# QZ1-boy/FCVSR

Hardware: AMD Instinct MI355X
Metric: SR frames/sec (7-frame window, 4x 180x320->720x1280) + PSNR vs ref (higher is better)
Workload: dtype bf16

## Files before the change

fcvsr_amd/csrc/iac.hip:

```cpp
#include "common.h"
#include "mfma_util.h"

namespace fcvsr {

typedef __attribute__((ext_vector_type(4))) float f32x4v_t;

constexpr int kIY = 4, kIX = 16, kIC = 32;
constexpr int kIHX = kIX + 2, kIHY = kIY + 2;

template <int KDT>
__device__ __forceinline__ void load_k12(const void* base, long long elem_off, float k[4][3]) {
  if (KDT == FCVSR_F32) {
    const float4* p = reinterpret_cast<const float4*>(reinterpret_cast<const float*>(base) + elem_off);
    const float4 a = p[0], b = p[1], c = p[2];
    k[0][0] = a.x; k[0][1] = a.y; k[0][2] = a.z; k[1][0] = a.w; k[1][1] = b.x; k[1][2] = b.y;
    k[2][0] = b.z; k[2][1] = b.w; k[2][2] = c.x; k[3][0] = c.y; k[3][1] = c.z; k[3][2] = c.w;
  } else {
    const uint2* p = reinterpret_cast<const uint2*>(reinterpret_cast<const uint16_t*>(base) + elem_off);
    const uint2 a = p[0], b = p[1], c = p[2];
    const unsigned w[6] = {a.x, a.y, b.x, b.y, c.x, c.y};
    float f[12];
#pragma unroll
    for (int i = 0; i < 6; ++i) {
      if (KDT == FCVSR_BF16) {
// ... 493 lines not shown
          for (int c = 0; c < 8; ++c) acc[c] = fmaf(v[c], k[c * 3 + tt], acc[c]);
        }
#pragma unroll
        for (int c = 0; c < 8; ++c) {
          acc[c] += f[c];
          acc[c] = acc[c] >= 0.f ? acc[c] : acc[c] * slope;
        }
        st_p8<ADT>(dst.p, (long long)b * dst.sb + (long long)gy * dst.sy + (long long)gx * dst.sx + c0, acc);
      }
    }
  };

  issue_taps(0);
  if (FK) {
    predictor_gemm();
    __syncthreads();
#pragma unroll
    for (int j = 0; j < 2; ++j) {
      const int p = j * 32 + ps;
      const uint4* kq = reinterpret_cast<const uint4*>(kt_s + ((p >> 4) * kIHX + (p & 15) + 1) * kKtRow + oct * 24);
      kin[j].q[0] = kq[0]; kin[j].q[1] = kq[1]; kin[j].q[2] = kq[2];
    }
    if (ps < 8) {
      const uint4* kq = reinterpret_cast<const uint4*>(kt_s + ((ps >> 1) * kIHX + ((ps & 1) ? kIHX - 1 : 0)) * kKtRow + oct * 24);
      khal.q[0] = kq[0]; khal.q[1] = kq[1]; khal.q[2] = kq[2];
    }
    __syncthreads();
  }
  warp_store(0);
  if (ND > 1) { issue_taps(1); issue_fin(1); }
  if (t + 1 < t_end) off_next = load_off(t + 1, tid);
  __syncthreads();
  sac_phases(0);
  if (ND > 1) {
    warp_store(1);
    __syncthreads();
    sac_phases(1);
  }
  }
}


constexpr int kQX = 14, kQVX = 16, kQY = 4, kQSY = kQY + 2;
constexpr int kQNS = kQSY * kQVX, kQNV = kQY * kQVX;

template <bool BF16>
__device__ __forceinline__ f32x4v_t mfma16x(uint4 a, uint4 b, f32x4v_t c) {
  if (BF16)
    return __builtin_amdgcn_mfma_f32_16x16x32_bf16(__builtin_bit_cast(bf16x8_t, a), __builtin_bit_cast(bf16x8_t, b), c, 0, 0, 0);
  else
    return __builtin_amdgcn_mfma_f32_16x16x32_f16(__builtin_bit_cast(f16x8_t, a), __builtin_bit_cast(f16x8_t, b), c, 0, 0, 0);
}

struct Iac2Args {
  const uint16_t* prev[2];
  const float* off[2];
  const uint16_t* fin[2];
  uint16_t* dst[2];
  const uint16_t* k0;
  const uint16_t* wk;
  const float* kbias;
  long long prev_sb, off_sb, fin_sb, dst_sb, k0_sb;
  int prev_sy, prev_sx, off_sy, off_sx, off_sc, fin_sy, fin_sx, dst_sy, dst_sx, k0_sy, k0_sx;
  float slope;
  int H, W, tiles_x, tiles_y, ntiles;
};

#ifndef FCVSR_IAC2_WGS
#define FCVSR_IAC2_WGS 3
#endif
template <int KDT, int ADT>
__global__ __launch_bounds__(256, FCVSR_IAC2_WGS) void iac_fused2_kernel(Iac2Args a) {
  constexpr int NG = 1;
  static_assert(ADT != FCVSR_F32 && KDT != FCVSR_F32, "16-bit form");
  constexpr bool BF = KDT == FCVSR_BF16;
  constexpr int SPP = 32 * NG;
  constexpr int ND = 2, NP = (kQNS + SPP - 1) / SPP;
  constexpr int EARLY = 2;
  __shared__ __align__(16) float s_all[kQNS * kJC];
  __shared__ __align__(16) uint16_t w_s[3 * kJC * kJC];
  __shared__ __align__(16) float kb_s[3 * kJC];
  const float slope = a.slope;
  const int H = a.H, W = a.W, tiles_x = a.tiles_x, tiles_y = a.tiles_y;
  int t_begin, t_end;
  {
    const int g = blockIdx.x, nwg = gridDim.x, qq = nwg >> 3, rr = nwg & 7, xcd = g & 7, loc = g >> 3;
    const int ci = (xcd < rr ? xcd * (qq + 1) : rr * (qq + 1) + (xcd - rr) * qq) + loc;
    t_begin = (int)((long long)ci * a.ntiles / nwg);
    t_end = (int)((long long)(ci + 1) * a.ntiles / nwg);
  }
  {
    const int tid = threadIdx.x;
#pragma unroll
    for (int i = 0; i < 3 * kJC * kJC / 8 / (256 * NG); ++i) {
      const int idx = tid + 256 * NG * i, R = idx >> 3, seg = idx & 7;
      const int mt = R >> 4, r = R & 15, tp = mt >> 2, cb = mt & 3;
      const int orig = ((r >> 2) * 16 + cb * 4 + (r & 3)) * 3 + tp;
      *reinterpret_cast<uint4*>(w_s + R * kJC + ((seg ^ (R & 7)) << 3)) = *reinterpret_cast<const uint4*>(a.wk + orig * kJC + seg * 8);
    }
    if (tid < 3 * kJC) {
      const int mt = tid >> 4, r = tid & 15, tp = mt >> 2, cb = mt & 3;
      kb_s[tid] = a.kbias[((r >> 2) * 16 + cb * 4 + (r & 3)) * 3 + tp];
    }
    __syncthreads();
  }
  auto load_off = [&](const int tt, const int tidv) {
    const int lanev = tidv & 63, wavev = tidv >> 6;
    const int bb = tt / (tiles_x * tiles_y), tt2 = tt - bb * tiles_x * tiles_y;
    const int oy0 = (tt2 / tiles_x) * kQY, ox0 = (tt2 % tiles_x) * kQX;
    const int sdir = lanev >> 5, sit = (lanev >> 3) & 3, spl = lanev & 7;
    int hp = sit * SPP + wavev * 8 + spl;
    hp = hp < kQNS ? hp : kQNS - 1;
    const int hy = hp >> 4, hx = hp & 15;
    int gy = oy0 + hy - 1, gx = ox0 + hx - 1;
    gy = gy < 0 ? 0 : (gy > H - 1 ? H - 1 : gy);
    gx = gx < 0 ? 0 : (gx > W - 1 ? W - 1 : gx);
    const float* op = (sdir ? a.off[1] : a.off[0]) + (long long)bb * a.off_sb + (gy * a.off_sy + gx * a.off_sx);
    return make_float2(op[0], op[a.off_sc]);
  };
  const int wave_s = __builtin_amdgcn_readfirstlane((int)threadIdx.x >> 6);
  float* const s_s = s_all;
  float* const v_s = s_s;
  float2 off_next = make_float2(0.f, 0.f);
  if (t_begin < t_end) off_next = load_off(t_begin, (int)threadIdx.x);
  for (int t = t_begin; t < t_end; ++t) {
    int tid;
    asm volatile("v_mbcnt_lo_u32_b32 %0, -1, 0\n\tv_mbcnt_hi_u32_b32 %0, -1, %0\n\tv_lshl_add_u32 %0, %1, 6, %0" : "=&v"(tid) : "s"(wave_s));
    auto fresh = [&]() { int x = tid; asm volatile("" : "+v"(x)); return x; };
    const int wave = wave_s;
    const int b = t / (tiles_x * tiles_y);
    const int t2 = t - b * tiles_x * tiles_y;
    const int ty0 = (t2 / tiles_x) * kQY, tx0 = (t2 % tiles_x) * kQX;
    const int row = ty0 + wave;
    const int rowc = row > H - 1 ? H - 1 : row;
    auto col_of = [&](const int n_) { const int x = tx0 + n_ - 1; return x < 0 ? 0 : (x > W - 1 ? W - 1 : x); };
    auto ld16 = [](const void* base, const unsigned byte_off) {
      Pack8<ADT> r;
      r.a = *reinterpret_cast<const uint4*>(reinterpret_cast<const char*>(base) + byte_off);
      r.b = make_uint4(0, 0, 0, 0);
      return r;
    };
    uint4 kfr[2];
    {
      const int x = fresh(), n = x & 15, q = (x & 63) >> 4;
      const uint16_t* kb = a.k0 + (long long)b * a.k0_sb + (long long)rowc * a.k0_sy;
      const unsigned e = (unsigned)(col_of(n) * a.k0_sx + q * 8) * 2u;
      kfr[0] = ld16(kb, e).a;
      kfr[1] = ld16(kb, e + 64u).a;
    }
    int my_eo[4];
    float my_w[4];
    {
      const int x = fresh(), lane = x & 63;
      const int sit = (lane >> 3) & 3, spl = lane & 7;
      int hp = sit * SPP + wave * 8 + spl;
      hp = hp < kQNS ? hp : kQNS - 1;
      const int hy = hp >> 4, hx = hp & 15;
      int gy = ty0 + hy - 1, gx = tx0 + hx - 1;
      gy = gy < 0 ? 0 : (gy > H - 1 ? H - 1 : gy);
      gx = gx < 0 ? 0 : (gx > W - 1 ? W - 1 : gx);
      const int psy = a.prev_sy, psx = a.prev_sx;
      const float fx = (float)gx + off_next.x;
      const float fy = (float)gy + off_next.y;
      const float x0f = floorf(fx), y0f = floorf(fy);
      const float wx1 = fx - x0f, wy1 = fy - y0f;
      const float wx0 = 1.f - wx1, wy0 = 1.f - wy1;
      int wb, hb;
      asm volatile("v_mov_b32 %0, %2\n\tv_mov_b32 %1, %3" : "=&v"(wb), "=&v"(hb) : "s"(W + 1), "s"(H + 1));
      const bool sane = (fx > -2.f) && (fx < (float)wb) && (fy > -2.f) && (fy < (float)hb);
      const int x0 = sane ? (int)x0f : -4, y0 = sane ? (int)y0f : -4;
#pragma unroll
      for (int dy = 0; dy < 2; ++dy) {
#pragma unroll
        for (int dx = 0; dx < 2; ++dx) {
          const int xi = x0 + dx, yi = y0 + dy;
          const bool in = xi >= 0 && xi < W && yi >= 0 && yi < H;
          const int xc = xi < 0 ? 0 : (xi > W - 1 ? W - 1 : xi), yc = yi < 0 ? 0 : (yi > H - 1 ? H - 1 : yi);
          my_w[dy * 2 + dx] = in ? (dy ? wy1 : wy0) * (dx ? wx1 : wx0) : 0.f;
          my_eo[dy * 2 + dx] = yc * psy + xc * psx;
        }
      }
    }
    __builtin_amdgcn_sched_barrier(0);
    Pack8<ADT> fpk[2];
    auto issue_fin = [&](const int dir) {
      const int x = fresh(), n = x & 15, q = (x & 63) >> 4;
      const uint16_t* fb = a.fin[dir] + (long long)b * a.fin_sb + (long long)rowc * a.fin_sy;
      const unsigned e = (unsigned)(col_of(n) * a.fin_sx + q * 16) * 2u;
      fpk[0] = ld16(fb, e);
      fpk[1] = ld16(fb, e + 16u);
    };
    Pack8<ADT> tap[ND][NP][4];
    auto issue_taps = [&](const int dir, const int it0, const int it1) {
      const int x = fresh(), oct = x & 7, pull = ((x & 63) >> 3) << 2;
      const uint16_t* pb = a.prev[dir] + (long long)b * a.prev_sb;
#pragma unroll
      for (int it = it0; it < it1; ++it) {
        const int src = pull + dir * 128 + it * 32;
#pragma unroll
        for (int k = 0; k < 4; ++k)
          tap[dir][it][k] = ld16(pb, (unsigned)(__builtin_amdgcn_ds_bpermute(src, my_eo[k]) + oct * 8) * 2u);
      }
    };
    auto warp_store = [&](const int dir) {
      const int x = fresh(), oct = x & 7, ps = x >> 3, pull = ((x & 63) >> 3) << 2;
#pragma unroll
      for (int it = 0; it < NP; ++it) {
        const int hp = it * SPP + ps;
        const int src = pull + dir * 128 + it * 32;
        float acc[8] = {0.f, 0.f, 0.f, 0.f, 0.f, 0.f, 0.f, 0.f};
        float tw[4];
#pragma unroll
        for (int k = 0; k < 4; ++k) tw[k] = __int_as_float(__builtin_amdgcn_ds_bpermute(src, __float_as_int(my_w[k])));
#pragma unroll
        for (int k = 0; k < 4; ++k) {
          float v[8];
          unpack8<ADT>(tap[dir][it][k], v);
          const float w = tw[k];
#pragma unroll
          for (int c = 0; c < 8; ++c) acc[c] = fmaf(v[c], w, acc[c]);
        }
        float* rec = s_s + hp * kJC;
        if (kQNS % SPP == 0 || hp < kQNS) {
          *reinterpret_cast<float4*>(rec + (((2 * oct) ^ (hp & 15)) << 2)) = make_float4(acc[0], acc[1], acc[2], acc[3]);
          *reinterpret_cast<float4*>(rec + (((2 * oct + 1) ^ (hp & 15)) << 2)) = make_float4(acc[4], acc[5], acc[6], acc[7]);
        }
        __builtin_amdgcn_sched_barrier(0);
      }
    };
    issue_taps(0, 0, NP);
    __builtin_amdgcn_sched_barrier(0);
    constexpr bool KF = NG == 1 && BF;
    uint2 K1p[KF ? 1 : 12];
    float K1f[KF ? 12 : 1][4];
    {
      const int x = fresh(), n = x & 15, q = (x & 63) >> 4;
#pragma unroll
      for (int mt = 0; mt < 12; ++mt) {
        const int R = mt * 16 + n;
        const uint4 w0 = *reinterpret_cast<const uint4*>(w_s + R * kJC + ((q ^ (R & 7)) << 3));
        const uint4 w1 = *reinterpret_cast<const uint4*>(w_s + R * kJC + (((q + 4) ^ (R & 7)) << 3));
        f32x4v_t acc = {0.f, 0.f, 0.f, 0.f};
        acc = mfma16x<BF>(w0, kfr[0], acc);
        acc = mfma16x<BF>(w1, kfr[1], acc);
        const float4 b4 = *reinterpret_cast<const float4*>(kb_s + mt * 16 + q * 4);
        const uint2 pk = cvt4<BF>(make_float4(acc[0] + b4.x, acc[1] + b4.y, acc[2] + b4.z, acc[3] + b4.w));
        if (KF) cvt16x4_to_f32<BF>(pk, K1f[mt]);
        else K1p[mt] = pk;
        if (mt & 1) __builtin_amdgcn_sched_barrier(0);
      }
    }
    int ov[4], oh[3][4];
    {
      const int x = fresh(), n = x & 15, q = (x & 63) >> 4;
#pragma unroll
      for (int cb = 0; cb < 4; ++cb) {
        ov[cb] = n * kJC + (((q * 4 + cb) ^ n) << 2);
#pragma unroll
        for (int tt = 0; tt < 3; ++tt) {
          const int m = n + tt - 1;
          oh[tt][cb] = m * kJC + (((q * 4 + cb) ^ (m & 15)) << 2);
        }
      }
    }
    auto sac = [&](const int dir) {
      float4 vr[4];
      {
#pragma unroll
        for (int cb = 0; cb < 4; ++cb) {
          float acc[4] = {0.f, 0.f, 0.f, 0.f};
#pragma unroll
          for (int tt = 0; tt < 3; ++tt) {
            const float4 sv = *reinterpret_cast<const float4*>(s_s + (wave + tt) * (kQVX * kJC) + ov[cb]);
            float k[4];
            if (KF) { k[0] = K1f[tt * 4 + cb][0]; k[1] = K1f[tt * 4 + cb][1]; k[2] = K1f[tt * 4 + cb][2]; k[3] = K1f[tt * 4 + cb][3]; }
            else cvt16x4_to_f32<BF>(K1p[tt * 4 + cb], k);
            acc[0] = fmaf(sv.x, k[0], acc[0]); acc[1] = fmaf(sv.y, k[1], acc[1]);
            acc[2] = fmaf(sv.z, k[2], acc[2]); acc[3] = fmaf(sv.w, k[3], acc[3]);
          }
          vr[cb] = make_float4(acc[0], acc[1], acc[2], acc[3]);
          __builtin_amdgcn_sched_barrier(0);
        }
      }
      issue_fin(dir);
      __syncthreads();
#pragma unroll
      for (int cb = 0; cb < 4; ++cb) *reinterpret_cast<float4*>(v_s + wave * (kQVX * kJC) + ov[cb]) = vr[cb];
      __syncthreads();
      const int x = fresh(), n = x & 15, q = (x & 63) >> 4;
      const int gx = tx0 + n - 1;
      if (n >= 1 && n <= kQX && row < H && gx < W) {
        uint16_t* const db = a.dst[dir] + (long long)b * a.dst_sb + (long long)row * a.dst_sy;
        const int e = gx * a.dst_sx + q * 16;
#pragma unroll
        for (int hf = 0; hf < 2; ++hf) {
          float f[8], o[8];
          unpack8<ADT>(fpk[hf], f);
#pragma unroll
          for (int c2 = 0; c2 < 2; ++c2) {
            const int cb = hf * 2 + c2;
            float acc[4] = {0.f, 0.f, 0.f, 0.f};
#pragma unroll
            for (int tt = 0; tt < 3; ++tt) {
              const float4 vv = *reinterpret_cast<const float4*>(v_s + wave * (kQVX * kJC) + oh[tt][cb]);
              float k[4];
              if (KF) { k[0] = K1f[tt * 4 + cb][0]; k[1] = K1f[tt * 4 + cb][1]; k[2] = K1f[tt * 4 + cb][2]; k[3] = K1f[tt * 4 + cb][3]; }
              else cvt16x4_to_f32<BF>(K1p[tt * 4 + cb], k);
              acc[0] = fmaf(vv.x, k[0], acc[0]); acc[1] = fmaf(vv.y, k[1], acc[1]);
              acc[2] = fmaf(vv.z, k[2], acc[2]); acc[3] = fmaf(vv.w, k[3], acc[3]);
            }
#pragma unroll
            for (int i = 0; i < 4; ++i) {
              const float r = acc[i] + f[c2 * 4 + i];
              o[c2 * 4 + i] = fmaxf(r, r * slope);
            }
          }
          st_p8<ADT>(reinterpret_cast<float*>(db), e + hf * 8, o);
          __builtin_amdgcn_sched_barrier(0);
        }
      }
    };
    __builtin_amdgcn_sched_barrier(0);
    warp_store(0);
    __builtin_amdgcn_sched_barrier(0);
    issue_taps(1, 0, EARLY);
    __builtin_amdgcn_sched_barrier(0);
    __syncthreads();
    sac(0);
    issue_taps(1, EARLY, NP);
    if (t + 1 < t_end) off_next = load_off(t + 1, fresh());
    __builtin_amdgcn_sched_barrier(0);
    __syncthreads();
    warp_store(1);
    __syncthreads();
    sac(1);
    __syncthreads();
  }
}

}

using namespace fcvsr;

static bool quad_ok(const fcvsr_view* v, int dt) {
  if (!v || !v->ptr || v->dtype != dt || v->sc != 1 || v->c % 4) return false;
  const int g = dt == FCVSR_F32 ? 4 : 4;
  const int al = dt == FCVSR_F32 ? 16 : 8;
  return v->sx % g == 0 && v->sy % g == 0 && v->sb % g == 0 && ((uintptr_t)v->ptr % al) == 0;
}

static int iac_persistent_wgs() {
  static int n[64] = {0};
  int dev = 0;
  if (hipGetDevice(&dev) != hipSuccess || dev < 0 || dev >= 64) return 512;
  if (!n[dev]) {
    hipDeviceProp_t prop;
    n[dev] = hipGetDeviceProperties(&prop, dev) == hipSuccess && prop.multiProcessorCount > 0 ? 2 * prop.multiProcessorCount : 512;
  }
  return n[dev];
}

template <int KDT, int ND, bool FK = false>
static void launch_iac64(int adt, dim3 grid, hipStream_t st, IacArgs a) {
  a.ntiles = (int)grid.x;
  if (FK) {
    int nwg = iac_persistent_wgs() / (int)grid.y;
    nwg = nwg < 8 ? 8 : nwg / 8 * 8;
    if (nwg < (int)grid.x) grid.x = nwg;
  }
  if (adt == FCVSR_F32) hipLaunchKernelGGL((iac_step64_kernel<KDT, FCVSR_F32, ND, FK>), grid, dim3(256), 0, st, a);
  else if (adt == FCVSR_BF16) hipLaunchKernelGGL((iac_step64_kernel<KDT, FCVSR_BF16, ND, FK>), grid, dim3(256), 0, st, a);
  else hipLaunchKernelGGL((iac_step64_kernel<KDT, FCVSR_F16, ND, FK>), grid, dim3(256), 0, st, a);
}

template <int KDT>
static void launch_iac(int adt, bool wide, dim3 grid, hipStream_t st, View pv, View ov, View kv, View fv, float slope, int B, int H,
                       int W, View dv, int tx, int ty) {
  if (wide) {
    IacArgs a;
    a.d[0].prev = pv; a.d[0].off = ov; a.d[0].fin = fv; a.d[0].dst = dv;
    a.d[1] = a.d[0];
    a.k1 = kv; a.k0 = kv; a.wk = nullptr; a.kbias = nullptr; a.slope = slope; a.B = B; a.H = H; a.W = W; a.tiles_x = tx; a.tiles_y = ty;
    launch_iac64<KDT, 1>(adt, grid, st, a);
    return;
  }
  if (adt == FCVSR_F32)
    hipLaunchKernelGGL((iac_step_kernel<KDT, FCVSR_F32>), grid, dim3(256), 0, st, pv, ov, kv, fv, slope, B, H, W, dv, tx, ty);
  else if (adt == FCVSR_BF16)
    hipLaunchKernelGGL((iac_step_kernel<KDT, FCVSR_BF16>), grid, dim3(256), 0, st, pv, ov, kv, fv, slope, B, H, W, dv, tx, ty);
  else
    hipLaunchKernelGGL((iac_step_kernel<KDT, FCVSR_F16>), grid, dim3(256), 0, st, pv, ov, kv, fv, slope, B, H, W, dv, tx, ty);
}

extern "C" int fcvsr_iac_step(const fcvsr_view* prev, const fcvsr_view* off, const fcvsr_view* k1, const fcvsr_view* feat_in,
                              float slope, int B, int H, int W, const fcvsr_view* dst, void* stream) {
  FCVSR_CHECK_ARG(prev && prev->ptr, "null prev");
  const int adt = prev->dtype;
  FCVSR_CHECK_ARG(adt == FCVSR_F32 || adt == FCVSR_BF16 || adt == FCVSR_F16, "bad feature dtype");
  FCVSR_CHECK_ARG(quad_ok(prev, adt) && quad_ok(feat_in, adt) && quad_ok(dst, adt),
                  "prev/feat_in/dst: same dtype, channel-contiguous, aligned");
  FCVSR_CHECK_ARG(off && off->ptr && off->c >= 2 && off->dtype == FCVSR_F32, "off needs 2 f32 channels");
  FCVSR_CHECK_ARG(k1 && k1->ptr && k1->sc == 1 && k1->c == 3 * prev->c, "k1 must have 3*C contiguous channels");
  FCVSR_CHECK_ARG(prev->c % kIC == 0 && prev->c == dst->c && prev->c == feat_in->c, "C must be a multiple of 32");
  FCVSR_CHECK_ARG(B > 0 && H > 0 && W > 0, "bad sizes");
  const int g = k1->dtype == FCVSR_F32 ? 4 : 8;
  FCVSR_CHECK_ARG(((uintptr_t)k1->ptr % 16) == 0 && k1->sx % g == 0 && k1->sy % g == 0 && k1->sb % g == 0, "k1 alignment");
  const int tx = cdiv(W, kIX), ty = cdiv(H, kIY);
  const int fa = adt == FCVSR_F32 ? 4 : 8;
  auto wide_ok = [&](const fcvsr_view* v) { return ((uintptr_t)v->ptr % 16) == 0 && v->sx % fa == 0 && v->sy % fa == 0 && v->sb % fa == 0; };
  const bool wide = prev->c % kJC == 0 && wide_ok(prev) && wide_ok(feat_in) && wide_ok(dst) &&
                    (long long)H * prev->sy < (1ll << 31);
  dim3 grid(B * tx * ty, prev->c / (wide ? kJC : kIC));
  hipStream_t st = (hipStream_t)stream;
  const View pv = to_view(*prev), ov = to_view(*off), kv = to_view(*k1), fv = to_view(*feat_in), dv = to_view(*dst);
  if (k1->dtype == FCVSR_F32) launch_iac<FCVSR_F32>(adt, wide, grid, st, pv, ov, kv, fv, slope, B, H, W, dv, tx, ty);
  else if (k1->dtype == FCVSR_BF16) launch_iac<FCVSR_BF16>(adt, wide, grid, st, pv, ov, kv, fv, slope, B, H, W, dv, tx, ty);
  else launch_iac<FCVSR_F16>(adt, wide, grid, st, pv, ov, kv, fv, slope, B, H, W, dv, tx, ty);
  FCVSR_LAUNCH_CHECK();
  return 0;
}

extern "C" int fcvsr_iac_step2(const fcvsr_view* prev, const fcvsr_view* off, const fcvsr_view* k1, const fcvsr_view* feat_in,
                               float slope, int B, int H, int W, const fcvsr_view* dst, void* stream) {
  FCVSR_CHECK_ARG(prev && off && k1 && feat_in && dst && prev[0].ptr, "null argument");
  const int adt = prev[0].dtype;
  FCVSR_CHECK_ARG(adt == FCVSR_F32 || adt == FCVSR_BF16 || adt == FCVSR_F16, "bad feature dtype");
  const int fa = adt == FCVSR_F32 ? 4 : 8;
  for (int d = 0; d < 2; ++d) {
    FCVSR_CHECK_ARG(quad_ok(&prev[d], adt) && quad_ok(&feat_in[d], adt) && quad_ok(&dst[d], adt),
                    "prev/feat_in/dst: same dtype, channel-contiguous, aligned");
    FCVSR_CHECK_ARG(off[d].ptr && off[d].c >= 2 && off[d].dtype == FCVSR_F32, "off needs 2 f32 channels");
    FCVSR_CHECK_ARG(prev[d].c % kJC == 0 && prev[d].c == prev[0].c && prev[d].c == dst[d].c && prev[d].c == feat_in[d].c,
                    "C must be a multiple of 64 and alike for both directions");
    const fcvsr_view* vs[3] = {&prev[d], &feat_in[d], &dst[d]};
    for (const fcvsr_view* v : vs)
      FCVSR_CHECK_ARG(((uintptr_t)v->ptr % 16) == 0 && v->sx % fa == 0 && v->sy % fa == 0 && v->sb % fa == 0,
                      "16-byte aligned feature views");
  }
  FCVSR_CHECK_ARG(k1->ptr && k1->sc == 1 && k1->c == 3 * prev[0].c, "k1 must have 3*C contiguous channels");
  FCVSR_CHECK_ARG(B > 0 && H > 0 && W > 0, "bad sizes");
  const int g = k1->dtype == FCVSR_F32 ? 4 : 8;
  FCVSR_CHECK_ARG(((uintptr_t)k1->ptr % 16) == 0 && k1->sx % g == 0 && k1->sy % g == 0 && k1->sb % g == 0, "k1 alignment");
  const int tx = cdiv(W, kIX), ty = cdiv(H, kIY);
  dim3 grid(B * tx * ty, prev[0].c / kJC);
  IacArgs a;
  for (int d = 0; d < 2; ++d) {
    a.d[d].prev = to_view(prev[d]); a.d[d].off = to_view(off[d]); a.d[d].fin = to_view(feat_in[d]); a.d[d].dst = to_view(dst[d]);
  }
  a.k1 = to_view(*k1); a.k0 = a.k1; a.wk = nullptr; a.kbias = nullptr; a.slope = slope; a.B = B; a.H = H; a.W = W; a.tiles_x = tx; a.tiles_y = ty;
  hipStream_t st = (hipStream_t)stream;
  if (k1->dtype == FCVSR_F32) launch_iac64<FCVSR_F32, 2>(adt, grid, st, a);
  else if (k1->dtype == FCVSR_BF16) launch_iac64<FCVSR_BF16, 2>(adt, grid, st, a);
  else if (k1->dtype == FCVSR_F16) launch_iac64<FCVSR_F16, 2>(adt, grid, st, a);
  else FCVSR_CHECK_ARG(false, "bad k1 dtype");
  FCVSR_LAUNCH_CHECK();
  return 0;
}

extern "C" int fcvsr_iac_step2_fused(const fcvsr_view* prev, const fcvsr_view* off, const fcvsr_view* k0, const void* wk,
                                     const float* kbias, const fcvsr_view* feat_in, float slope, int B, int H, int W,
                                     const fcvsr_view* dst, void* stream) {
  FCVSR_CHECK_ARG(prev && off && k0 && wk && kbias && feat_in && dst && prev[0].ptr, "null argument");
  const int adt = prev[0].dtype;
  FCVSR_CHECK_ARG(adt == FCVSR_F32 || adt == FCVSR_BF16 || adt == FCVSR_F16, "bad feature dtype");
  const int fa = adt == FCVSR_F32 ? 4 : 8;
  for (int d = 0; d < 2; ++d) {
    FCVSR_CHECK_ARG(quad_ok(&prev[d], adt) && quad_ok(&feat_in[d], adt) && quad_ok(&dst[d], adt),
                    "prev/feat_in/dst: same dtype, channel-contiguous, aligned");
    FCVSR_CHECK_ARG(off[d].ptr && off[d].c >= 2 && off[d].dtype == FCVSR_F32, "off needs 2 f32 channels");
    FCVSR_CHECK_ARG(prev[d].c == kJC && dst[d].c == kJC && feat_in[d].c == kJC, "the fused predictor handles C == 64");
    const fcvsr_view* vs[3] = {&prev[d], &feat_in[d], &dst[d]};
    for (const fcvsr_view* v : vs)
      FCVSR_CHECK_ARG(((uintptr_t)v->ptr % 16) == 0 && v->sx % fa == 0 && v->sy % fa == 0 && v->sb % fa == 0,
                      "16-byte aligned feature views");
  }
  FCVSR_CHECK_ARG(k0->ptr && (k0->dtype == FCVSR_BF16 || k0->dtype == FCVSR_F16) && k0->sc == 1 && k0->c == kJC &&
                      ((uintptr_t)k0->ptr % 16) == 0 && k0->sx % 8 == 0 && k0->sy % 8 == 0 && k0->sb % 8 == 0,
                  "k0: 64 contiguous 16-bit channels, 16-byte aligned");
  FCVSR_CHECK_ARG(((uintptr_t)wk % 16) == 0 && ((uintptr_t)kbias % 16) == 0, "weights / bias must be 16-byte aligned");
  FCVSR_CHECK_ARG(B > 0 && H > 0 && W > 0, "bad sizes");
  FCVSR_CHECK_ARG((long long)H * prev[0].sy < (1ll << 31) && (long long)H * prev[1].sy < (1ll << 31), "image too large");
  const int tx = cdiv(W, kIX), ty = cdiv(H, kIY);
  dim3 grid(B * tx * ty, 1);
  IacArgs a;
  for (int d = 0; d < 2; ++d) {
    a.d[d].prev = to_view(prev[d]); a.d[d].off = to_view(off[d]); a.d[d].fin = to_view(feat_in[d]); a.d[d].dst = to_view(dst[d]);
  }
  a.k1 = to_view(*k0); a.k0 = to_view(*k0); a.wk = (const uint16_t*)wk; a.kbias = kbias;
  a.slope = slope; a.B = B; a.H = H; a.W = W; a.tiles_x = tx; a.tiles_y = ty;
  hipStream_t st = (hipStream_t)stream;
  bool same = adt != FCVSR_F32 && adt == k0->dtype && (long long)H * k0->sy < (1ll << 31);
  {
    const fcvsr_view* sets[4] = {prev, off, feat_in, dst};
    for (const fcvsr_view* v : sets)
      same = same && v[0].sb == v[1].sb && v[0].sy == v[1].sy && v[0].sx == v[1].sx && v[0].sc == v[1].sc && (long long)H * v[0].sy < (1ll << 31);
  }
  if (same && slope >= 0.f && slope <= 1.f) {
    Iac2Args q;
    for (int d = 0; d < 2; ++d) {
      q.prev[d] = (const uint16_t*)prev[d].ptr; q.off[d] = (const float*)off[d].ptr;
      q.fin[d] = (const uint16_t*)feat_in[d].ptr; q.dst[d] = (uint16_t*)dst[d].ptr;
    }
    q.k0 = (const uint16_t*)k0->ptr; q.wk = (const uint16_t*)wk; q.kbias = kbias;
    q.prev_sb = prev[0].sb; q.off_sb = off[0].sb; q.fin_sb = feat_in[0].sb; q.dst_sb = dst[0].sb; q.k0_sb = k0->sb;
    q.prev_sy = (int)prev[0].sy; q.prev_sx = (int)prev[0].sx; q.off_sy = (int)off[0].sy; q.off_sx = (int)off[0].sx; q.off_sc = (int)off[0].sc;
    q.fin_sy = (int)feat_in[0].sy; q.fin_sx = (int)feat_in[0].sx; q.dst_sy = (int)dst[0].sy; q.dst_sx = (int)dst[0].sx;
    q.k0_sy = (int)k0->sy; q.k0_sx = (int)k0->sx;
    q.slope = slope; q.H = H; q.W = W; q.tiles_x = cdiv(W, kQX); q.tiles_y = cdiv(H, kQY); q.ntiles = B * q.tiles_x * q.tiles_y;
    int nwg = iac_persistent_wgs() / 2 * FCVSR_IAC2_WGS;
    nwg = nwg < 8 ? 8 : nwg / 8 * 8;
    if (nwg > q.ntiles) nwg = q.ntiles;
    if (adt == FCVSR_BF16) hipLaunchKernelGGL((iac_fused2_kernel<FCVSR_BF16, FCVSR_BF16>), dim3(nwg), dim3(256), 0, st, q);
    else hipLaunchKernelGGL((iac_fused2_kernel<FCVSR_F16, FCVSR_F16>), dim3(nwg), dim3(256), 0, st, q);
    FCVSR_LAUNCH_CHECK();
    return 0;
  }
  if (k0->dtype == FCVSR_BF16) launch_iac64<FCVSR_BF16, 2, true>(adt, grid, st, a);
  else launch_iac64<FCVSR_F16, 2, true>(adt, grid, st, a);
  FCVSR_LAUNCH_CHECK();
  return 0;
}
```

fcvsr_amd/hip.py:

```python
from __future__ import annotations

import ctypes as C
import os
from typing import Optional, Sequence

import numpy as np
import torch

_HERE = os.path.dirname(os.path.abspath(__file__))
LIB_PATH = os.path.join(_HERE, "lib", "libfcvsr_hip.so")

F32, BF16, F16, U8, U16 = 0, 1, 2, 3, 4
ACT_NONE, ACT_RELU, ACT_LEAKY, ACT_PRELU = 0, 1, 2, 3
_DT = {torch.float32: F32, torch.bfloat16: BF16, torch.float16: F16, torch.uint8: U8, torch.uint16: U16}


class View(C.Structure):
    _fields_ = [("ptr", C.c_void_p), ("sb", C.c_int64), ("sy", C.c_int64), ("sx", C.c_int64), ("sc", C.c_int64),
                ("c", C.c_int32), ("dtype", C.c_int32)]


class GcFinishLevel(C.Structure):
    _fields_ = [("partial", C.c_void_p), ("add", C.c_void_p), ("nparts", C.c_int32)]

# ... 52 lines not shown
                ("gc_wmask", C.c_void_p), ("gc_partial", C.c_void_p)]


PROFILE = None
COMPUTE_DTYPE = "f32"
DOMINANT_KERNEL = "conv_direct_kernel"


class HipError(RuntimeError):
    pass


_lib: Optional[C.CDLL] = None

_VP, _I, _I64, _F = C.c_void_p, C.c_int, C.c_int64, C.c_float
_PV = C.POINTER(View)
SIGNATURES = {
    "fcvsr_last_error": [],
    "fcvsr_last_conv_kernel": [],
    "fcvsr_conv2d_wgrad_scratch_elems": [C.c_int] * 7,
    "fcvsr_conv2d_wgrad": [C.c_void_p, C.c_void_p, C.c_int, C.c_int, C.c_int, C.c_int, C.c_int, C.c_int, C.c_int, C.c_void_p, C.c_void_p,
                           C.c_longlong, C.c_int, C.c_void_p],
    "fcvsr_conv2d_wgrad_mfma_eligible": [C.c_int] * 6,
    "fcvsr_conv2d_wgrad_mfma_scratch_elems": [C.c_int] * 7,
    "fcvsr_conv2d_wgrad_mfma": [C.c_void_p, C.c_void_p, C.c_int, C.c_int, C.c_int, C.c_int, C.c_int, C.c_int, C.c_int, C.c_void_p, C.c_void_p,
                                C.c_void_p, C.c_longlong, C.c_int, C.c_int, C.c_void_p],
    "fcvsr_abi_version": [],
    "fcvsr_device_count": [],
    "fcvsr_conv2d": [C.POINTER(ConvDesc), _VP],
    "fcvsr_conv2d_f32mfma": [C.POINTER(ConvDesc), _VP],
    "fcvsr_conv2d_f32mfma_eligible": [C.POINTER(ConvDesc)],
    "fcvsr_conv2d_mfma": [C.POINTER(ConvDesc), _I, _I, _VP],
    "fcvsr_conv2d_mfma_plan": [C.POINTER(ConvDesc), _I, _I, _I, _I, C.c_char_p, _I],
    "fcvsr_rfft2": [_PV, _I, _I, _I, _I, _VP, _I64, _I, _I, _VP],
    "fcvsr_irfft2": [_VP, _I64, _I, _I, _I, _I, _I, _I, _VP, _VP, _PV, _VP],
    "fcvsr_irfft2_bands": [_VP, _I64, _I, _I, _I, _I, _I, _I, _VP, _I, _VP, _PV, _VP],
    "fcvsr_last_fft_path": [],
    "fcvsr_corr_lookup": [_VP, _VP, _I64, _I, _I, _I, _I, _I, _I, _PV, _VP],
    "fcvsr_channel_sum": [_PV, _I, _I, _I, _VP, _VP, _I64, _VP],
    "fcvsr_ca_gate": [_VP, _F, _VP, _VP, _I, _I, _I, _VP, _VP],
    "fcvsr_convblk_tail": [_VP, _VP, _VP, _I, _I, _I, _I, _VP, _I64, _I, _I, _I, _I, _VP],
    "fcvsr_convblk": [_VP, _VP, _VP, _VP, _I, _VP, _VP, _VP, _I, _I, _I, _I, _VP, _VP, _I64, _VP, _I64, _I, _I, _I, _I, _VP],
    "fcvsr_convblk_heads": [_VP, _I, _VP, _VP, _VP, _VP, _VP, _VP, _I, _I, _I, _VP, _VP, _I64, _VP, _I64, _I, _I, _VP],
    "fcvsr_warp": [_PV, _PV, _I, _I, _I, _PV, _VP],
    "fcvsr_sac_v": [_PV, _PV, _I, _I, _I, _PV, _VP],
    "fcvsr_sac_h": [_PV, _PV, _PV, _F, _I, _I, _I, _PV, _VP],
    "fcvsr_iac_step": [_PV, _PV, _PV, _PV, _F, _I, _I, _I, _PV, _VP],
    "fcvsr_feat_extract": [_PV, _I, _I, _I, _VP, _VP, _I, _VP, _VP, _VP, _I, _VP],
    "fcvsr_freq_head": [_VP, _I, _I64, _I64, _VP, _VP, _VP, _VP, _VP],
    "fcvsr_convcorr_strip": [_VP, _VP, _I, _I, _I, _I, _VP, _VP, _VP, _VP, _VP],
    "fcvsr_freq_mlp3": [_VP, _VP, _I, _I64, _I64, _VP, _VP, _VP, _VP, _I64, _VP],
    "fcvsr_iac_step2": [_PV, _PV, _PV, _PV, _F, _I, _I, _I, _PV, _VP],
    "fcvsr_iac_step2_fused": [_PV, _PV, _PV, _VP, _VP, _PV, _F, _I, _I, _I, _PV, _VP],
    "fcvsr_divenh": [_I, _I, _VP, _VP, _VP, _VP, _VP, _VP, _F, _VP, _VP, _VP, _VP, _I64, _I, _I, _I, _I, _VP],
    "fcvsr_divenh_apply_next": [_I, _VP, _VP, _VP, _VP, _VP, _VP, _F, _VP, _VP, _VP, _VP, _VP, _VP, _VP, _I64, _I, _I, _I, _I, _VP],
    "fcvsr_divenh_stage": [C.POINTER(DivEnhStageArgs), _VP],
    "fcvsr_scale_add": [_VP, _VP, _VP, _I, _VP, _I, _I, _I, _I, _I, _VP],
    "fcvsr_gc_context": [_VP, _VP, _VP, _VP, _I, _I, _I, _I, _VP, _VP, _I64, _VP],
    "fcvsr_gc_finish": [_VP, _I, _VP, _VP, _I, _I, _VP, _VP],
    "fcvsr_gc_apply": [_VP, _VP, _VP, _VP, _I, _F, _I, _I, _I, _I, _VP],
    "fcvsr_xscale": [_VP, _VP, _F, _VP, _VP, _VP, _I, _I, _I, _I, _I, _VP],
    "fcvsr_gc_finish_levels": [C.POINTER(GcFinishLevel), _I, _VP, _VP, _I, _I, _VP],
    "fcvsr_gc_partial_levels": [C.POINTER(GcPartialLevel), _I, _I, _VP, _I, _VP],
    "fcvsr_gc_apply_levels": [C.POINTER(GcApplyLevel), _I, _I, _I, _F, _I, _VP],
    "fcvsr_xscale_levels": [C.POINTER(XscaleLevel), _I, _I, _I, _VP],
    "fcvsr_rcb_level0": [_VP, _VP, _VP, _VP, _VP, _VP, _VP, _F, _F, _I, _I, _I, _I, _I, _VP],
    "fcvsr_rcb_tail": [C.POINTER(RcbTailArgs), _F, _I, _I, _VP],
    "fcvsr_pixel_shuffle": [_VP, _VP, _I, _I, _I, _I, _VP],
    "fcvsr_pixel_shuffle16": [_VP, _PV, _I, _I, _I, _I, _VP],
    "fcvsr_bilinear_up4": [_PV, _I, _I, _I, _PV, _VP],
    "fcvsr_tail_fused": [_PV, _VP, _VP, _VP, _VP, _VP, _I, _I, _I, _PV, _VP],
    "fcvsr_tail_fused_base": [_PV, _VP, _VP, _VP, _VP, _VP, _PV, _I, _I, _I, _PV, _VP],
    "fcvsr_conv_last": [_PV, _VP, _VP, _I, _I, _I, _I, _PV, _VP],
    "fcvsr_pack_weight_mfma": [_VP, _I, _I, _I, _I, _VP, _I, _I, _I, _I, _VP],
    "fcvsr_pack_weights_multi_block_elems": [],
    "fcvsr_pack_weights_mfma_multi": [_VP, _I, _I, _I, _VP],
    "fcvsr_adam_multi_block_elems": [],
    "fcvsr_adam_multi": [_VP, _I, _I, _VP, _VP, _VP, _I, _F, _F, _F, _F, _F, _F, _F, _VP],
    "fcvsr_act_bwd": [_VP, _VP, _VP, _F, C.c_longlong, _VP],
    "fcvsr_colsum_scratch_elems": [C.c_longlong, _I],
    "fcvsr_colsum": [_VP, C.c_longlong, _I, _VP, _VP, C.c_longlong, _I, _VP],
    "fcvsr_iac_bwd_sac": [_VP, _VP, _VP, _VP, _PV, _F, _I, _I, _I, _I, _VP, _I, _VP, _PV, _I, _VP],
    "fcvsr_iac_bwd_warp": [_VP, _PV, _VP, _PV, _I, _I, _I, _I, _VP, _VP, _VP],
    "fcvsr_iac_bwd_warp_det_workspace": [_I, _I, _I, _I, C.POINTER(C.c_size_t)],
    "fcvsr_iac_bwd_warp_det": [_VP, _PV, _VP, _PV, _I, _I, _I, _I, _VP, _VP, _VP, C.c_size_t, _VP],
    "fcvsr_prelu_fwd": [_VP, _VP, _VP, C.c_longlong, _VP],
    "fcvsr_prelu_bwd": [_VP, _VP, _VP, _VP, _VP, _VP, C.c_longlong, _VP],
    "fcvsr_wgrad_cout1_scratch_elems": [_I, _I, _I],
    "fcvsr_wgrad_cout1": [_VP, _VP, _I, _I, _I, _I, _VP, _VP, C.c_longlong, _I, _VP],
    "fcvsr_conv2d_wgrad_mfma_groups_scratch_elems": [_VP, _VP, _VP, _I, _I, _I, _I, _I],
    "fcvsr_conv2d_wgrad_mfma_groups": [_VP, _VP, _VP, _VP, _VP, _I, _I, _I, _I, _VP, _VP, _VP, C.c_longlong, _I, _I, _VP],
    "fcvsr_up2_adjoint": [_VP, _VP, _I, _I, _I, _I, _VP],
    "fcvsr_pool2_adjoint": [_VP, _VP, _I, _I, _I, _I, _VP],
    "fcvsr_rcbt_nblk": [_I],
    "fcvsr_rcbt_stat_elems": [],
    "fcvsr_rcbt_forward": [_VP, _VP, _VP, _VP, _VP, _F, _I, _I, _I, _VP, _VP, _VP, C.c_longlong, _VP],
    "fcvsr_rcbt_backward": [_VP, _VP, _VP, _VP, _VP, _VP, _F, _I, _I, _I, _VP, _VP, _VP, _VP, _VP, C.c_longlong, _I, _VP],
    "fcvsr_divenh_band_nblk": [_I],
    "fcvsr_divenh_band_stat_elems": [_I],
    "fcvsr_divenh_band_forward": [_VP, _VP, _VP, _VP, _VP, _VP, _VP, _I, _I, _I, _VP, _VP, _VP, _VP, C.c_longlong, _VP],
    "fcvsr_divenh_band_backward": [_VP, _VP, _VP, _VP, _VP, _VP, _VP, _VP, _VP, _VP, _I, _I, _I, _VP, _VP, _VP, _VP, _VP, _VP, _VP, _VP,
                                   C.c_longlong, _I, _VP],
    "fcvsr_corr_lookup_bwd": [_VP, _VP, _I64, _I, _I, _I, _I, _I, _I, _PV, _VP, _VP, _VP],
    "fcvsr_frame_metrics_scratch_bytes": [_I] * 6,
    "fcvsr_frame_metrics": [_VP, C.POINTER(C.c_int64), _I, _VP, C.POINTER(C.c_int64), _I, _I, _I, _I, _I, _I,
                            C.POINTER(C.c_double), _VP, _VP, C.c_longlong, _VP],
# ... 506 lines not shown
```

include/fcvsr_hip.h:

```cpp
#ifndef FCVSR_HIP_H
#define FCVSR_HIP_H

#include <stddef.h>
#include <stdint.h>

#ifdef __cplusplus
extern "C" {
#endif

#define FCVSR_ABI_VERSION 2

enum { FCVSR_E_ARG = -1, FCVSR_E_UNSUPPORTED = -2, FCVSR_E_NOGPU = -3 };
enum { FCVSR_F32 = 0, FCVSR_BF16 = 1, FCVSR_F16 = 2 };
enum { FCVSR_U8 = 3 };
enum { FCVSR_U16 = 4 };
enum { FCVSR_ACT_NONE = 0, FCVSR_ACT_RELU = 1, FCVSR_ACT_LEAKY = 2, FCVSR_ACT_PRELU = 3 };

typedef struct fcvsr_view {
  void*   ptr;
  int64_t sb, sy, sx, sc;
  int32_t c;
  int32_t dtype;
} fcvsr_view;

// ... 76 lines not shown
                      int W, int C, float* gfin, int fin_accumulate, float* gv, const fcvsr_view* gk, int k_accumulate, void* stream);
int fcvsr_iac_bwd_warp(const float* gv, const fcvsr_view* k1, const float* prev, const fcvsr_view* off, int B, int H, int W, int C,
                       float* gprev_zeroed, float* goff, void* stream);
int fcvsr_iac_bwd_warp_det_workspace(int B, int H, int W, int C, size_t* bytes);
int fcvsr_iac_bwd_warp_det(const float* gv, const fcvsr_view* k1, const float* prev, const fcvsr_view* off, int B, int H, int W, int C,
                           float* gprev, float* goff, void* workspace, size_t workspace_bytes, void* stream);
long long fcvsr_conv2d_wgrad_mfma_groups_scratch_elems(const int* B, const int* H, const int* W, int n_groups, int cin, int cout, int kh,
                                                       int kw);
int fcvsr_conv2d_wgrad_mfma_groups(const fcvsr_view* xs, const fcvsr_view* gys, const int* B, const int* H, const int* W, int n_groups, int kh,
                                   int kw, int pad, float* dw, float* dbias, float* scratch, long long scratch_elems, int dw_accumulate,
                                   int dbias_accumulate, void* stream);
int fcvsr_up2_adjoint(const float* g, float* out, int B, int H, int W, int C, void* stream);
int fcvsr_pool2_adjoint(const float* g, float* out, int B, int H, int W, int C, void* stream);
int fcvsr_rfft2(const fcvsr_view* src, int B, int H, int W, int n,
                float* spec, int64_t pix_stride, int im_off, int re_off, void* stream);
int fcvsr_irfft2(const float* spec, int64_t pix_stride, int im_off, int re_off, int B, int H, int W, int n,
                 const float* mask, float* work, const fcvsr_view* dst, void* stream);
int fcvsr_irfft2_bands(const float* spec, int64_t pix_stride, int im_off, int re_off, int B, int H, int W, int n,
                       const float* masks, int n_bands, float* work, const fcvsr_view* dst, void* stream);
const char* fcvsr_last_fft_path(void);

int fcvsr_feat_extract(const fcvsr_view* x, int B, int H, int W, const void* w, const float* bias, int n_blk,
                       void* const* dst, const int64_t* dst_pix_stride, const int32_t* dst_ch_off, int dst_dtype,
                       void* stream);

int fcvsr_corr_lookup(const float* x1f, const float* x2f, int64_t pix_stride, int B, int H, int Wf, int C, int radius,
                      int x_count, const fcvsr_view* dst, void* stream);
int fcvsr_channel_sum(const fcvsr_view* src, int B, int H, int W, float* out, float* scratch, int64_t scratch_elems,
                      void* stream);
int fcvsr_ca_gate(const float* sum, float inv_hw, const float* w1, const float* w2, int B, int c, int cr,
                  float* gate, void* stream);
int fcvsr_convblk_tail(const float* u, const float* gate, const float* sim, int B, int ndir, int H, int Wf,
                       float* spec, int64_t pix_stride, int re_off, int im_off, int g_stride, int g0, void* stream);
int fcvsr_convblk(const float* x, const float* w1, const float* w2, const float* prelu_slope, int ksize, const float* ca_w1,
                  const float* ca_w2, const float* sim, int B, int ndir, int H, int Wf, float* u_scratch,
                  float* partial_scratch, int64_t partial_elems, float* spec, int64_t pix_stride, int re_off, int im_off,
                  int g_stride, int g0, void* stream);
int fcvsr_convblk_heads(const float* x, int n_heads, const float* const* w1, const float* const* w2,
                        const float* const* prelu_slope, const float* const* ca_w1, const float* const* ca_w2, const float* sim,
                        int B, int H, int Wf, float* u, float* partial, int64_t partial_elems, float* spec, int64_t pix_stride,
                        int re_off, int im_off, void* stream);
int fcvsr_warp(const fcvsr_view* src, const fcvsr_view* off, int B, int H, int W, const fcvsr_view* dst, void* stream);
int fcvsr_sac_v(const fcvsr_view* s, const fcvsr_view* k1, int B, int H, int W, const fcvsr_view* dst, void* stream);
int fcvsr_sac_h(const fcvsr_view* v, const fcvsr_view* k1, const fcvsr_view* feat_in, float slope,
                int B, int H, int W, const fcvsr_view* dst, void* stream);

int fcvsr_iac_step(const fcvsr_view* prev, const fcvsr_view* off, const fcvsr_view* k1, const fcvsr_view* feat_in,
                   float slope, int B, int H, int W, const fcvsr_view* dst, void* stream);
int fcvsr_iac_step2(const fcvsr_view* prev, const fcvsr_view* off, const fcvsr_view* k1, const fcvsr_view* feat_in,
                    float slope, int B, int H, int W, const fcvsr_view* dst, void* stream);
int fcvsr_iac_step2_fused(const fcvsr_view* prev, const fcvsr_view* off, const fcvsr_view* k0, const void* wk,
                          const float* kbias, const fcvsr_view* feat_in, float slope, int B, int H, int W,
                          const fcvsr_view* dst, void* stream);

int fcvsr_freq_mlp3(const float* const* xa, const float* const* xb, int n_dirs, int64_t src_pix_stride, int64_t npix,
                    const void* w0, const void* w2, const void* w4, void* const* dst, int64_t dst_pix_stride, void* stream);

int fcvsr_freq_head(const void* x, int x_dtype, int64_t x_pix_stride, int64_t npix, const void* w0, const void* w_mid,
                    const void* w_last, float* out, void* stream);
int fcvsr_convcorr_strip(const void* off, const float* corr, int B, int H, int Wf, int xs, const void* w0, const void* w_mid,
                         const void* w_last, float* off4, void* stream);

int fcvsr_divenh(int mode, int first, const float* f, float* s_f, float* s_o, const float* a, const float* b,
                 const float* mean_f_sum, float inv_hw, const float* g1, const float* g2,
                 float* sums, float* scratch, int64_t scratch_elems, int B, int H, int W, int C, void* stream);
int fcvsr_divenh_apply_next(int first, const float* f, float* s_f, float* s_o, const float* a, const float* b,
                            const float* mean_f_sum, float inv_hw, const float* g1, const float* g2,
                            const float* f_next, const float* a_next, const float* b_next, float* sums,
                            float* scratch, int64_t scratch_elems, int B, int H, int W, int C, void* stream);
typedef struct {
  const float* ck_s_f;
  const float* ck_s_o;
  const float* f[4];
  const float* a[4];
  const float* b[4];
  const float* g1[4];
  const float* g2[4];
  const float* mean_f_sum;
  const float* f_next;
  const float* a_next;
  const float* b_next;
  float*       out_s_f;
  float*       out_s_o;
  float*       sums;
  float*       scratch;
  int64_t      scratch_elems;
  float        inv_hw;
  int32_t      n_bands, B, H, W, C;
} fcvsr_divenh_stage_args;
int fcvsr_divenh_stage(const fcvsr_divenh_stage_args* a, void* stream);
int fcvsr_scale_add(const float* z, const float* gate, const void* x, int x_dtype, void* out, int out_dtype, int B, int H,
                    int W, int C, void* stream);

int fcvsr_gc_context(const float* r, const float* wmask, const float* w1, const float* w2, int B, int H, int W, int C,
                     float* add, float* scratch, int64_t scratch_elems, void* stream);
int fcvsr_gc_finish(const float* partial, int nparts, const float* w1, const float* w2, int B, int C, float* add,
                    void* stream);
int fcvsr_gc_apply(const float* r, const float* add, const void* z, void* out, int io_dtype, float slope,
                   int B, int H, int W, int C, void* stream);
int fcvsr_xscale(const void* x, const void* r, float r_scale, const void* dn, const void* up, void* out, int io_dtype,
                 int B, int H, int W, int C, void* stream);

typedef struct {
  const float* partial;
  float*       add;
  int32_t      nparts;
// ... 157 lines not shown
```

Measured before the change: 923.8.

## Walk fused IAC tiles down column strips and reuse the warped halo row

The fused IAC kernel now orders tiles column-strip-major: each workgroup steps down vertical strips and carries the last warped halo row of the previous tile in registers. It writes that row back into shared memory as the new top halo, so the first halo pass of gathers and bilinear blends is skipped on continuation tiles. A workgroup-count cap is also added through a new _wgs entry point, which defaults to off. The cost is extra registers for the kept rows and a dependence on consecutive tiles within a workgroup sharing a strip, which also changes the memory access order.

```diff
diff --git a/fcvsr_amd/csrc/iac.hip b/fcvsr_amd/csrc/iac.hip
--- a/fcvsr_amd/csrc/iac.hip
+++ b/fcvsr_amd/csrc/iac.hip
@@ -569,6 +569,9 @@
     return __builtin_amdgcn_mfma_f32_16x16x32_f16(__builtin_bit_cast(f16x8_t, a), __builtin_bit_cast(f16x8_t, b), c, 0, 0, 0);
 }
 
+template <bool V>
+struct BoolTag { static constexpr bool value = V; };
+
 struct Iac2Args {
   const uint16_t* prev[2];
   const float* off[2];
@@ -624,8 +627,11 @@
   auto load_off = [&](const int tt, const int tidv) {
     const int lanev = tidv & 63, wavev = tidv >> 6;
     const int bb = tt / (tiles_x * tiles_y), tt2 = tt - bb * tiles_x * tiles_y;
-    const int oy0 = (tt2 / tiles_x) * kQY, ox0 = (tt2 % tiles_x) * kQX;
-    const int sdir = lanev >> 5, sit = (lanev >> 3) & 3, spl = lanev & 7;
+    const int strip = tt2 / tiles_y, step = tt2 - strip * tiles_y;
+    const int oy0 = step * kQY, ox0 = strip * kQX;
+    const int sdir = lanev >> 5, spl = lanev & 7;
+    int sit = (lanev >> 3) & 3;
+    if (tt != t_begin && step > 0) sit = sit ? sit : 1;
     int hp = sit * SPP + wavev * 8 + spl;
     hp = hp < kQNS ? hp : kQNS - 1;
     const int hy = hp >> 4, hx = hp & 15;
@@ -640,14 +646,20 @@
   float* const v_s = s_s;
   float2 off_next = make_float2(0.f, 0.f);
   if (t_begin < t_end) off_next = load_off(t_begin, (int)threadIdx.x);
-  for (int t = t_begin; t < t_end; ++t) {
+  float4 keep[ND][2];
+#pragma unroll
+  for (int d = 0; d < ND; ++d) keep[d][0] = keep[d][1] = make_float4(0.f, 0.f, 0.f, 0.f);
+  auto tile = [&](const int t, auto cont_tag) {
+    constexpr bool cont = decltype(cont_tag)::value;
+    constexpr int p0 = cont ? 1 : 0;
     int tid;
     asm volatile("v_mbcnt_lo_u32_b32 %0, -1, 0\n\tv_mbcnt_hi_u32_b32 %0, -1, %0\n\tv_lshl_add_u32 %0, %1, 6, %0" : "=&v"(tid) : "s"(wave_s));
     auto fresh = [&]() { int x = tid; asm volatile("" : "+v"(x)); return x; };
     const int wave = wave_s;
     const int b = t / (tiles_x * tiles_y);
     const int t2 = t - b * tiles_x * tiles_y;
-    const int ty0 = (t2 / tiles_x) * kQY, tx0 = (t2 % tiles_x) * kQX;
+    const int strip = t2 / tiles_y, step = t2 - strip * tiles_y;
+    const int ty0 = step * kQY, tx0 = strip * kQX;
     const int row = ty0 + wave;
     const int rowc = row > H - 1 ? H - 1 : row;
     auto col_of = [&](const int n_) { const int x = tx0 + n_ - 1; return x < 0 ? 0 : (x > W - 1 ? W - 1 : x); };
@@ -713,18 +725,26 @@
       const uint16_t* pb = a.prev[dir] + (long long)b * a.prev_sb;
 #pragma unroll
       for (int it = it0; it < it1; ++it) {
-        const int src = pull + dir * 128 + it * 32;
-#pragma unroll
-        for (int k = 0; k < 4; ++k)
-          tap[dir][it][k] = ld16(pb, (unsigned)(__builtin_amdgcn_ds_bpermute(src, my_eo[k]) + oct * 8) * 2u);
+        if (it + p0 < NP) {
+          const int src = pull + dir * 128 + (it + p0) * 32;
+#pragma unroll
+          for (int k = 0; k < 4; ++k)
+            tap[dir][it][k] = ld16(pb, (unsigned)(__builtin_amdgcn_ds_bpermute(src, my_eo[k]) + oct * 8) * 2u);
+        }
       }
     };
     auto warp_store = [&](const int dir) {
       const int x = fresh(), oct = x & 7, ps = x >> 3, pull = ((x & 63) >> 3) << 2;
+      if (cont) {
+        float* rec = s_s + ps * kJC;
+        *reinterpret_cast<float4*>(rec + (((2 * oct) ^ (ps & 15)) << 2)) = keep[dir][0];
+        *reinterpret_cast<float4*>(rec + (((2 * oct + 1) ^ (ps & 15)) << 2)) = keep[dir][1];
+      }
 #pragma unroll
       for (int it = 0; it < NP; ++it) {
-        const int hp = it * SPP + ps;
-        const int src = pull + dir * 128 + it * 32;
+        if (it + p0 >= NP) continue;
+        const int hp = (it + p0) * SPP + ps;
+        const int src = pull + dir * 128 + (it + p0) * 32;
         float acc[8] = {0.f, 0.f, 0.f, 0.f, 0.f, 0.f, 0.f, 0.f};
         float tw[4];
 #pragma unroll
@@ -798,6 +818,12 @@
           vr[cb] = make_float4(acc[0], acc[1], acc[2], acc[3]);
           __builtin_amdgcn_sched_barrier(0);
         }
+      }
+      {
+        const int x = fresh(), oct = x & 7, ps = x >> 3;
+        const float* rec = s_s + (4 * kQVX + ps) * kJC;
+        keep[dir][0] = *reinterpret_cast<const float4*>(rec + (((2 * oct) ^ (ps & 15)) << 2));
+        keep[dir][1] = *reinterpret_cast<const float4*>(rec + (((2 * oct + 1) ^ (ps & 15)) << 2));
       }
       issue_fin(dir);
       __syncthreads();
@@ -852,6 +878,10 @@
     __syncthreads();
     sac(1);
     __syncthreads();
+  };
+  for (int t = t_begin; t < t_end; ++t) {
+    if (t != t_begin && t % tiles_y != 0) tile(t, BoolTag<true>{});
+    else tile(t, BoolTag<false>{});
   }
 }
 
@@ -878,12 +908,13 @@
 }
 
 template <int KDT, int ND, bool FK = false>
-static void launch_iac64(int adt, dim3 grid, hipStream_t st, IacArgs a) {
+static void launch_iac64(int adt, dim3 grid, hipStream_t st, IacArgs a, int max_wgs = 0) {
   a.ntiles = (int)grid.x;
   if (FK) {
     int nwg = iac_persistent_wgs() / (int)grid.y;
     nwg = nwg < 8 ? 8 : nwg / 8 * 8;
     if (nwg < (int)grid.x) grid.x = nwg;
+    if (max_wgs > 0 && max_wgs < (int)grid.x) grid.x = max_wgs;
   }
   if (adt == FCVSR_F32) hipLaunchKernelGGL((iac_step64_kernel<KDT, FCVSR_F32, ND, FK>), grid, dim3(256), 0, st, a);
   else if (adt == FCVSR_BF16) hipLaunchKernelGGL((iac_step64_kernel<KDT, FCVSR_BF16, ND, FK>), grid, dim3(256), 0, st, a);
@@ -977,6 +1008,13 @@
 extern "C" int fcvsr_iac_step2_fused(const fcvsr_view* prev, const fcvsr_view* off, const fcvsr_view* k0, const void* wk,
                                      const float* kbias, const fcvsr_view* feat_in, float slope, int B, int H, int W,
                                      const fcvsr_view* dst, void* stream) {
+  return fcvsr_iac_step2_fused_wgs(prev, off, k0, wk, kbias, feat_in, slope, B, H, W, dst, 0, stream);
+}
+
+extern "C" int fcvsr_iac_step2_fused_wgs(const fcvsr_view* prev, const fcvsr_view* off, const fcvsr_view* k0, const void* wk,
+                                         const float* kbias, const fcvsr_view* feat_in, float slope, int B, int H, int W,
+                                         const fcvsr_view* dst, int max_workgroups, void* stream) {
+  FCVSR_CHECK_ARG(max_workgroups >= 0, "max_workgroups: 0 (default) or a positive cap");
   FCVSR_CHECK_ARG(prev && off && k0 && wk && kbias && feat_in && dst && prev[0].ptr, "null argument");
   const int adt = prev[0].dtype;
   FCVSR_CHECK_ARG(adt == FCVSR_F32 || adt == FCVSR_BF16 || adt == FCVSR_F16, "bad feature dtype");
@@ -1027,13 +1065,14 @@
     int nwg = iac_persistent_wgs() / 2 * FCVSR_IAC2_WGS;
     nwg = nwg < 8 ? 8 : nwg / 8 * 8;
     if (nwg > q.ntiles) nwg = q.ntiles;
+    if (max_workgroups > 0 && nwg > max_workgroups) nwg = max_workgroups;
     if (adt == FCVSR_BF16) hipLaunchKernelGGL((iac_fused2_kernel<FCVSR_BF16, FCVSR_BF16>), dim3(nwg), dim3(256), 0, st, q);
     else hipLaunchKernelGGL((iac_fused2_kernel<FCVSR_F16, FCVSR_F16>), dim3(nwg), dim3(256), 0, st, q);
     FCVSR_LAUNCH_CHECK();
     return 0;
   }
-  if (k0->dtype == FCVSR_BF16) launch_iac64<FCVSR_BF16, 2, true>(adt, grid, st, a);
-  else launch_iac64<FCVSR_F16, 2, true>(adt, grid, st, a);
+  if (k0->dtype == FCVSR_BF16) launch_iac64<FCVSR_BF16, 2, true>(adt, grid, st, a, max_workgroups);
+  else launch_iac64<FCVSR_F16, 2, true>(adt, grid, st, a, max_workgroups);
   FCVSR_LAUNCH_CHECK();
   return 0;
 }
diff --git a/fcvsr_amd/hip.py b/fcvsr_amd/hip.py
--- a/fcvsr_amd/hip.py
+++ b/fcvsr_amd/hip.py
@@ -128,6 +128,7 @@
     "fcvsr_freq_mlp3": [_VP, _VP, _I, _I64, _I64, _VP, _VP, _VP, _VP, _I64, _VP],
     "fcvsr_iac_step2": [_PV, _PV, _PV, _PV, _F, _I, _I, _I, _PV, _VP],
     "fcvsr_iac_step2_fused": [_PV, _PV, _PV, _VP, _VP, _PV, _F, _I, _I, _I, _PV, _VP],
+    "fcvsr_iac_step2_fused_wgs": [_PV, _PV, _PV, _VP, _VP, _PV, _F, _I, _I, _I, _PV, _I, _VP],
     "fcvsr_divenh": [_I, _I, _VP, _VP, _VP, _VP, _VP, _VP, _F, _VP, _VP, _VP, _VP, _I64, _I, _I, _I, _I, _VP],
     "fcvsr_divenh_apply_next": [_I, _VP, _VP, _VP, _VP, _VP, _VP, _F, _VP, _VP, _VP, _VP, _VP, _VP, _VP, _I64, _I, _I, _I, _I, _VP],
     "fcvsr_divenh_stage": [C.POINTER(DivEnhStageArgs), _VP],
diff --git a/include/fcvsr_hip.h b/include/fcvsr_hip.h
--- a/include/fcvsr_hip.h
+++ b/include/fcvsr_hip.h
@@ -152,6 +152,9 @@
 int fcvsr_iac_step2_fused(const fcvsr_view* prev, const fcvsr_view* off, const fcvsr_view* k0, const void* wk,
                           const float* kbias, const fcvsr_view* feat_in, float slope, int B, int H, int W,
                           const fcvsr_view* dst, void* stream);
+int fcvsr_iac_step2_fused_wgs(const fcvsr_view* prev, const fcvsr_view* off, const fcvsr_view* k0, const void* wk,
+                              const float* kbias, const fcvsr_view* feat_in, float slope, int B, int H, int W,
+                              const fcvsr_view* dst, int max_workgroups, void* stream);
 
 int fcvsr_freq_mlp3(const float* const* xa, const float* const* xb, int n_dirs, int64_t src_pix_stride, int64_t npix,
                     const void* w0, const void* w2, const void* w4, void* const* dst, int64_t dst_pix_stride, void* stream);
```

Result: no change. 929.3 (median of 6 runs) (+0.6%).
